# jatinchowdhury18/differentiable-wdfs

Hardware: AMD Instinct MI355X
Metric: samples/sec fwd+bwd, 1N4148 diode clipper @48kHz batch=8192; 1->8 GPU scaling (higher is better)
Workload: dtype f32

## Files before the change

### differentiable-wdfs_amd/csrc/wdf_clipper.h

```cpp
#pragma once

#include <hip/hip_runtime.h>
#include <stdint.h>
#include <type_traits>

#include "wdf_omega.h"
#include "wdf_optim.h"

namespace wdf {

#ifdef WDF_DBG_TIMES
__device__ unsigned long long* g_dbg_times = nullptr;
#define WDF_DBG_STAMP(i)                                                                                     \
    do { if (threadIdx.x == 0 && g_dbg_times)                                                                \
             g_dbg_times[8 * ((size_t)gridDim.x * gridDim.y) + 8 * (size_t)blockIdx.x + (i)] = wall_clock64(); } while (0)
#else
#define WDF_DBG_STAMP(i) do {} while (0)
#endif

constexpr int kBlk = 8;

struct ClipConsts {
    float Is, V;
    float G2;
// ... 78 lines not shown
}

template <int NSTEP, bool VEC4>
__device__ __forceinline__ void load_row(const float* __restrict__ x, int64_t b, int64_t T, int64_t t0,
                                         float (&v)[NSTEP])
{
    if constexpr (VEC4) {
        const float4* p = reinterpret_cast<const float4*>(x + b * T + t0);
#pragma unroll
        for (int i = 0; i < NSTEP / 4; ++i) {
            const float4 f = p[i];
            v[4 * i] = f.x; v[4 * i + 1] = f.y; v[4 * i + 2] = f.z; v[4 * i + 3] = f.w;
        }
    } else {
#pragma unroll
        for (int k = 0; k < NSTEP; ++k) v[k] = x[b * T + t0 + k];
    }
}

template <bool TIME_MAJOR>
__device__ __forceinline__ float load_one(const float* __restrict__ x, int64_t b, int64_t B, int64_t T, int64_t t)
{
    return TIME_MAJOR ? x[t * B + b] : x[b * T + t];
}

__device__ __forceinline__ bool series_only_omega1(const ClipConsts& c)
{
    return c.L - fminf(c.d.l_up, c.d.l_dn) <= kSeriesOnlyBelow;
}

template <int DYN_R>
__device__ __forceinline__ bool fast_root_ok(const ClipConsts& c, int general)
{
    if (general) return false;
    if constexpr (DYN_R) return (c.lIV - logf(c.G2)) - fminf(c.d.l_up, c.d.l_dn) <= kSeriesOnlyBelow;
    else return series_only_omega1(c);
}

template <int DYN_R, bool SYM>
__device__ __forceinline__ int root_tier(const ClipConsts& c, int general)
{
    if (!fast_root_ok<DYN_R>(c, general)) return kRootGeneral;
    if constexpr (SYM && !DYN_R) {
        const float l0 = c.L - c.d.l_dn;
        if (l0 <= -7.5f && l0 >= -80.0f) return kRootLean;
    }
    if constexpr (SYM && DYN_R == 2) {
        const float lmax = (c.lIV - logf(c.G2)) - c.d.l_dn;
        if (lmax <= -7.5f && c.lIV >= -50.0f) return kRootLean;
    }
    return kRootFast;
}

template <int DYN_R, bool SYM, typename V, int FAST = 0>
__device__ __forceinline__ V fwd_step(const ClipConsts& c, V xin, V rin, V& z)
{
    V p, Rp, L;
    step_coeffs<DYN_R, V>(c, rin, p, Rp, L);
    const V b_diff = z - xin;
    const V b_temp = -p * b_diff;
    const V a = z + b_temp;
    const DiodeOutT<V> o = diode_pair<SYM, V, FAST>(a, L, c.d);
    const V zn = o.b + b_temp;
    const V y = 0.5f * (zn + z);
    z = zn;
    return y;
}

template <int DYN_R, bool SYM, bool TIME_MAJOR, bool VEC4, bool STASH, int FAST>
__device__ __forceinline__ void clipper_fwd_body(const ClipConsts& c, const float* __restrict__ x,
                                                 const float* __restrict__ r, float* __restrict__ y,
                                                 float* __restrict__ zstash, const float* __restrict__ z0,
                                                 float* __restrict__ zT, int64_t B, int64_t T)
{
    const int64_t b_raw = (int64_t)blockIdx.x * 64 + threadIdx.x;
    const int64_t b = b_raw < B ? b_raw : B - 1;
    float z = z0 ? z0[b] : 0.0f;
    float* __restrict__ yp = y + b;
    float* __restrict__ zp = STASH ? zstash + b : nullptr;

    const int64_t nfull = T / kBlk;
    float xc[kBlk], xn[kBlk], rc[kBlk], rn[kBlk];
#pragma unroll
    for (int k = 0; k < kBlk; ++k) { xc[k] = xn[k] = 0.0f; rc[k] = rn[k] = 1.0f; }
    if (nfull > 0) {
        load_block<TIME_MAJOR, VEC4>(x, b, B, T, 0, xn);
        if constexpr (DYN_R) load_block<TIME_MAJOR, VEC4>(r, b, B, T, 0, rn);
    }
    for (int64_t blk = 0; blk < nfull; ++blk) {
        const int64_t t0 = blk * kBlk;
#pragma unroll
        for (int k = 0; k < kBlk; ++k) { xc[k] = xn[k]; if constexpr (DYN_R) rc[k] = rn[k]; }
        if (blk + 1 < nfull) {
            load_block<TIME_MAJOR, VEC4>(x, b, B, T, t0 + kBlk, xn);
            if constexpr (DYN_R) load_block<TIME_MAJOR, VEC4>(r, b, B, T, t0 + kBlk, rn);
        }
#pragma unroll
        for (int k = 0; k < kBlk; ++k) {
            if constexpr (STASH) { *zp = z; zp += B; }
            *yp = fwd_step<DYN_R, SYM, float, FAST>(c, xc[k], rc[k], z);
            yp += B;
        }
    }
    for (int64_t t = nfull * kBlk; t < T; ++t) {
        const float xin = load_one<TIME_MAJOR>(x, b, B, T, t);
        const float rin = DYN_R ? load_one<TIME_MAJOR>(r, b, B, T, t) : 1.0f;
        if constexpr (STASH) { *zp = z; zp += B; }
        *yp = fwd_step<DYN_R, SYM, float, FAST>(c, xin, rin, z);
        yp += B;
    }
    if (zT) zT[b] = z;
}

template <int DYN_R, bool SYM, bool TIME_MAJOR, bool VEC4, bool STASH>
__global__ __launch_bounds__(64) void clipper_fwd_kernel(
// ... 1051 lines not shown
```

### differentiable-wdfs_amd/csrc/wdf_clipper_fused.h

```cpp
#pragma once

#include "wdf_clipper.h"
#include "wdf_esr.h"

namespace wdf {

constexpr int kFsOut = 5;
constexpr int kFsOutEsr = 6;
constexpr int kFsPart = 4;
constexpr int kFsPartEsr = 8;
template <int LOSS> struct FusedRec {
    static constexpr int N = LOSS == 2 ? kFsOutEsr : kFsOut;
    static constexpr int NP = LOSS == 2 ? kFsPartEsr : kFsPart;
};
constexpr int kFsQuads = 3;
template <int NSEQ, int LOSS> struct FusedQuads { static constexpr int NQ = (NSEQ * FusedRec<LOSS>::N + 3) / 4; };
__device__ __forceinline__ float* rec_chunk(float* rec, int64_t k) { return rec + (size_t)k * kFsQuads * ((size_t)gridDim.x * 64) * 4; }
constexpr int kFusedSchedGroup = 1;
#ifndef WDF_FUSED_ROWS
#define WDF_FUSED_ROWS 16
#endif
#ifndef WDF_FUSED_PREFETCH_AT
#define WDF_FUSED_PREFETCH_AT 0
#endif
// ... 238 lines not shown
        const int g = threadIdx.x & 3, lr = threadIdx.x >> 2;
        commit(a);
#pragma unroll
        for (int m = 0; m < N * 2; ++m)
            *reinterpret_cast<v4u*>(lds + (o * HR + m * 16 + lr) * kWinPitch + kWinPhase + g * 4) = tail[m];
        read(tw, v);
        if (N == 1 && tw + NR < t_end) issue(o, tw + NR);
    }
    __device__ __forceinline__ void next(int64_t tn, int64_t t_end, V (&v)[NR])
    {
        const int sel = (int)(tn / kWinPhase) & 1, u = (int)(tn / NR) % N;
        if (u == 0) commit(sel);
        read(tn, v);
        if (u == N - 1 && tn + NR < t_end) issue(sel ^ 1, tn + NR);
    }
};

template <typename V>
__device__ __forceinline__ V load_own(const float* row, const LaneOwn<V>& q)
{
    V r = vsplat<V>(0.0f);
#pragma unroll
    for (int j = 0; j < VT<V>::N; ++j) vset(r, j, row[q.b + j]);
    return r;
}
template <typename V>
__device__ __forceinline__ void store_own(float* row, const LaneOwn<V>& q, V v)
{
#pragma unroll
    for (int j = 0; j < VT<V>::N; ++j) row[q.b + j] = vget(v, j);
}
template <typename V>
__device__ __forceinline__ void publish_own(float* row, const LaneOwn<V>& q, V v)
{
#pragma unroll
    for (int j = 0; j < VT<V>::N; ++j) __hip_atomic_store(row + q.b + j, vget(v, j), __ATOMIC_RELAXED, __HIP_MEMORY_SCOPE_AGENT);
}
template <typename V, bool TM>
__device__ __forceinline__ V load_step(const float* __restrict__ x, const LaneOwn<V>& q, int64_t B, int64_t T, int64_t t)
{
    V r = vsplat<V>(0.0f);
#pragma unroll
    for (int j = 0; j < VT<V>::N; ++j) vset(r, j, load_one<TM>(x, q.b + j, B, T, t));
    return r;
}

template <typename V>
struct FusedTan {
    V A, cL, cV, cP;
    V GA, GL, GV, GP;
    V hg_prev;
    V sse;
    V HA, HL, HV, HP, hy_prev, syy;
    __device__ __forceinline__ void init()
    {
        A = vsplat<V>(1.0f);
        cL = cV = cP = GA = GL = GV = GP = hg_prev = sse = vsplat<V>(0.0f);
        HA = HL = HV = HP = hy_prev = syy = vsplat<V>(0.0f);
    }
    template <int LOSS>
    __device__ __forceinline__ void pin()
    {
        vpin(A); vpin(cL); vpin(cV); vpin(cP); vpin(GA); vpin(GL); vpin(GV); vpin(GP); vpin(sse);
        if constexpr (LOSS == 2) { vpin(HA); vpin(HL); vpin(HV); vpin(HP); vpin(syy); }
    }
};

template <int DYN_R, bool SYM, int FAST, typename V, int LOSS = 1>
__device__ __forceinline__ V fused_step(const ClipConsts& c, V xin, V rin, V tgt, float hgs, V& z, FusedTan<V>& s)
{
    V p, Rp, L;
    step_coeffs<DYN_R, V>(c, rin, p, Rp, L);
    const V b_diff = z - xin;
    const V b_temp = -p * b_diff;
    const V a = z + b_temp;
    const DiodeOutT<V> o = diode_pair<SYM, V, FAST>(a, L, c.d);
    const V zn = o.b + b_temp;
    const V y = 0.5f * (zn + z);
    const V w0p = o.w0 * vrcp(o.w0 + 1.0f);
    V Da, DL, DV;
    if constexpr (SYM && FAST == kRootLean && !DYN_R) {
        const V w1p = vfma(-o.w1, o.w1, o.w1);
        const V sp = w0p + w1p;
        const V tl = vsel_nonzero(a, -2.0f, 0.0f);
        const float tvm = c.d.two_v * c.d.m_dn;
        Da = vfma(tl, sp, 1.0f);
        DL = vcopysign(w0p - w1p, a);
        DV = vfma(tl * a, sp, tvm * vcopysign(o.dw, a));
        const V cPl = vfma(-Da, b_diff, -b_diff);
        const V kappa_l = vfma(Da, 1.0f - c.p, -c.p);
        const V d = y - tgt;
        const V hg = hgs * d;
        s.sse = vfma(hg, d, s.sse);
        const V hh = hg + s.hg_prev;
        s.hg_prev = hg;
        s.GA = vfma(hh, s.A, s.GA);
        s.GL = vfma(hh, s.cL, s.GL);
        s.GV = vfma(hh, s.cV, s.GV);
        s.GP = vfma(hh, s.cP, s.GP);
        if constexpr (LOSS == 2) {
            const V hy = hgs * y;
            s.syy = vfma(hy, y, s.syy);
            const V h2 = hy + s.hy_prev;
            s.hy_prev = hy;
            s.HA = vfma(h2, s.A, s.HA);
            s.HL = vfma(h2, s.cL, s.HL);
            s.HV = vfma(h2, s.cV, s.HV);
            s.HP = vfma(h2, s.cP, s.HP);
        }
        s.A = s.A * kappa_l;
        s.cL = vfma(kappa_l, s.cL, DL);
        s.cV = vfma(kappa_l, s.cV, DV);
        s.cP = vfma(kappa_l, s.cP, cPl);
        z = zn;
        return y;
    } else
    if constexpr (SYM && FAST) {
        V w1p;
        if constexpr (FAST == kRootLean) w1p = vfma(-o.w1, o.w1, o.w1);
        else w1p = o.w1 * vfma(-o.w1, vfma(-o.w1, 1.0f - o.w1, 1.0f), 1.0f);
        const V sp = w0p + w1p;
        const V tl = vsel_nonzero(a, -2.0f, 0.0f);
        const float tvm = c.d.two_v * c.d.m_dn;
        Da = vfma(tl, sp, 1.0f);
        DL = (-tvm) * vcopysign(w0p - w1p, a);
        DV = vfma(tl * a, sp * (-1.0f / c.V), (-2.0f * c.d.m_dn) * vcopysign(o.dw, a));
    } else {
        const V w1p = o.w1 * vrcp(o.w1 + 1.0f);
        const V l2 = o.lam * o.lam;
        const V sp = w0p + w1p;
        const V tl = -2.0f * l2;
        Da = vfma(tl, sp, 1.0f);
        if constexpr (SYM) {
            const float tvm = c.d.two_v * c.d.m_dn;
            DL = (-tvm) * (o.lam * (w0p - w1p));
            DV = vfma(tl * a, sp * (-1.0f / c.V), (-2.0f * c.d.m_dn) * (o.lam * (o.w0 - o.w1)));
        } else {
            DL = (-c.d.two_v) * (o.lam * (o.m0 * w0p - o.m1 * w1p));
            DV = vfma(tl * a, sp * (-1.0f / c.V), -2.0f * (o.lam * (o.m0 * o.w0 - o.m1 * o.w1)));
        }
    }
    const V opd = Da + 1.0f;
    V cP = -opd * b_diff;
    if constexpr (DYN_R) cP = Rp * vfma(cP, p, DL);
    const V kappa = vfma(-p, opd, Da);
    const V d = y - tgt;
    const V hg = hgs * d;
    s.sse = vfma(hg, d, s.sse);
    const V hh = hg + s.hg_prev;
    s.hg_prev = hg;
    s.GA = vfma(hh, s.A, s.GA);
    s.GL = vfma(hh, s.cL, s.GL);
    s.GV = vfma(hh, s.cV, s.GV);
    s.GP = vfma(hh, s.cP, s.GP);
    if constexpr (LOSS == 2) {
        const V hy = hgs * y;
        s.syy = vfma(hy, y, s.syy);
        const V h2 = hy + s.hy_prev;
        s.hy_prev = hy;
        s.HA = vfma(h2, s.A, s.HA);
        s.HL = vfma(h2, s.cL, s.HL);
        s.HV = vfma(h2, s.cV, s.HV);
        s.HP = vfma(h2, s.cP, s.HP);
    }
    s.A = s.A * kappa;
    s.cL = vfma(kappa, s.cL, DL);
// ... 109 lines not shown
    int64_t t0, t1;
    chunk_span(k, K, L, skew, T, t0, t1);
    int64_t tw = 0;
    V z = vsplat<V>(0.0f);
    TpCtl c0 = {};
    if (ctl != nullptr) c0 = *ctl;
    __builtin_amdgcn_sched_barrier(0);
    const bool stateful = ctl != nullptr && c0.geom == tp_geom_tag(K, J, tp_span_scheme(skew));
    const int valid = stateful ? c0.valid : 0;
    const int head = stateful ? c0.head : 0;
    const bool warm_start = k > 0 && valid > 0 && !(stateful && c0.cold_hold > 0);
    const int jw = warm_start ? c0.j_next : 0;
    if (warm_start) tw = t0 - (int64_t)kWarmStep * jw;
    else tw = (t0 > W) ? t0 - W : 0;
    float* __restrict__ snapw = (snap != nullptr && k + 1 < K) ? snap + ((int64_t)((head + 1) % kTpRing) * J * K + k) * B : nullptr;

    const uint32_t rowb = (uint32_t)B * 4u;
    const uint32_t boff = q.boff;
    V xc[NR], xn[NR], rc[NR], rn[NR], gc[NR], gn[NR];
#pragma unroll
    for (int i = 0; i < NR; ++i) { xc[i] = xn[i] = gc[i] = gn[i] = vsplat<V>(0.0f); rc[i] = rn[i] = vsplat<V>(1.0f); }
    const int64_t nfull_end = t1 - (t1 - tw) % NR;
    constexpr bool WIN = fused_x_window<DYN_R, TM, VEC4>();
    XWindow<V, WIN> xw(x, q, B, T);
    if constexpr (WIN) static_assert(NR == XWindow<V, true>::NR, "a window is N tiles");
    if (tw < nfull_end) {
        if constexpr (WIN) xw.first_issue(tw);
        else load_x_tile<V, TM, VEC4, NR>(x, q, B, T, tw, rowb, xn);
        if constexpr (DYN_R == 1) load_x_tile<V, TM, VEC4, NR>(r, q, B, T, tw, rowb, rn);
        if constexpr (LOSS != 0) { if (tw >= t0) load_rows<V, NR>(target + tw * B, boff, rowb, gn); }
    }
    if (warm_start) {
        const int h2 = valid > 1 ? (head + kTpRing - 1) % kTpRing : head;
        const int h3 = valid > 2 ? (head + kTpRing - 2) % kTpRing : h2;
        z = load_own<V>(snap + (((int64_t)head * J + jw) * K + (k - 1)) * B, q);
        const V z2 = load_own<V>(snap + (((int64_t)h2 * J + jw) * K + (k - 1)) * B, q);
        const V z3 = load_own<V>(snap + (((int64_t)h3 * J + jw) * K + (k - 1)) * B, q);
        __builtin_amdgcn_sched_barrier(0);
        if (valid > 1) {
            const TpExtrap e = tp_extrapolation(theta, c0, valid);
            const V zs = vfma(vsplat<V>(e.lam), z - z2, z);
            if (e.quad) {
                const V zq = vfma(vsplat<V>(e.w3), z3 - z, vfma(vsplat<V>(e.w2), z2 - z, z));
                const V c = zq - zs;
                z = zs + vsel(vgt_c(vabs(c), 4.0e-7f), c, vsplat<V>(0.0f));
            } else {
                z = zs;
            }
        }
    } else if (tw == 0 && z0) {
        z = load_own<V>(z0, q);
    }
    int64_t t = tw;
    if constexpr (WIN) { if (tw < nfull_end) xw.first(tw, nfull_end, xn); }
#ifdef WDF_DBG_TIMES
    dbg_p[1] = __builtin_amdgcn_s_memtime();
#endif
    for (; t < t0 && t < nfull_end; t += NR) {
#pragma unroll
        for (int i = 0; i < NR; ++i) { xc[i] = xn[i]; if constexpr (DYN_R == 1) rc[i] = rn[i]; }
        if (t + NR < nfull_end) {
            if constexpr (WIN) xw.next(t + NR, nfull_end, xn);
            else load_x_tile<V, TM, VEC4, NR>(x, q, B, T, t + NR, rowb, xn);
            if constexpr (DYN_R == 1) load_x_tile<V, TM, VEC4, NR>(r, q, B, T, t + NR, rowb, rn);
            if constexpr (LOSS != 0) { if (t + NR >= t0) load_rows<V, NR>(target + (t + NR) * B, boff, rowb, gn); }
        }
#pragma unroll
        for (int i = 0; i < NR; ++i) (void)fwd_step<DYN_R, SYM, V, FAST>(c, xc[i], rc[i], z);
    }
#ifdef WDF_DBG_TIMES
    dbg_p[2] = __builtin_amdgcn_s_memtime();
#endif
    publish_own<V>(zwarm + k * B, q, z);
    if (gs != nullptr) {
#pragma unroll
        for (int j = 0; j < VT<V>::N; ++j) gs->zin[j][threadIdx.x & 63u] = vget(z, j);
    }
    wait_vmcnt<0>();
#ifdef WDF_DBG_TIMES
    dbg_p[3] = __builtin_amdgcn_s_memtime();
#endif
    FusedTan<V> s;
    s.init();
    FusedSums<V> d;
    d.init();
#ifdef WDF_DBG_TIMES
    unsigned long long dbg_wait = 0;
#endif
    for (; t < nfull_end; t += NR) {
#pragma unroll
        for (int i = 0; i < NR; ++i) { xc[i] = xn[i]; gc[i] = gn[i]; if constexpr (DYN_R == 1) rc[i] = rn[i]; }
        const bool more = t + NR < nfull_end;
        if (snapw != nullptr && t1 - t <= (int64_t)kWarmStep * (J - 1) && (t1 - t) % kWarmStep == 0)
            store_own<V>(snapw + ((t1 - t) / kWarmStep) * K * B, q, z);
        [[maybe_unused]] const __amdgpu_buffer_rsrc_t ry = row_rsrc(STORE_Y ? y + t * B : nullptr);
        [[maybe_unused]] const __amdgpu_buffer_rsrc_t rz = row_rsrc(STASH ? zstash + t * B : (STORE_Y ? y + t * B : nullptr));
        const int64_t below = skip - t;
        const int n_masked = __builtin_amdgcn_readfirstlane((int)(below < 0 ? 0 : (below > NR ? NR : below)));
#pragma unroll
        for (int i = 0; i < NR; ++i) {
            if (i == kFusedPrefetchAt * NR / 2) {
                __builtin_amdgcn_sched_barrier(0);
                if (more) {
                    if constexpr (WIN) xw.next(t + NR, nfull_end, xn);
                    else load_x_tile<V, TM, VEC4, NR>(x, q, B, T, t + NR, rowb, xn);
                    if constexpr (DYN_R == 1) load_x_tile<V, TM, VEC4, NR>(r, q, B, T, t + NR, rowb, rn);
                    if constexpr (LOSS != 0) load_rows<V, NR>(target + (t + NR) * B, boff, rowb, gn);
                }
                __builtin_amdgcn_sched_barrier(0);
            }
            if constexpr (LOSS == 0) {
                if constexpr (STASH) buf_store_nt(z, rz, boff, i * rowb);
                buf_store_nt(fwd_step<DYN_R, SYM, V, FAST>(c, xc[i], rc[i], z), ry, boff, i * rowb);
                continue;
            }
            if constexpr (STORE_Y)
                buf_store_nt(fused_step<DYN_R, SYM, FAST, V, LOSS>(c, xc[i], rc[i], gc[i], step_loss_scale(i, n_masked, hgs), z, s), ry, boff,
                             i * rowb);
            else
                (void)fused_step<DYN_R, SYM, FAST, V, LOSS>(c, xc[i], rc[i], gc[i], step_loss_scale(i, n_masked, hgs), z, s);
            if (i % kFusedSchedGroup == kFusedSchedGroup - 1) {
                s.template pin<LOSS>();
                __builtin_amdgcn_sched_barrier(0);
            }
        }
#ifdef WDF_DBG_TIMES
        { const unsigned long long w0 = __builtin_amdgcn_s_memtime(); wait_vmcnt<NR>(); dbg_wait += __builtin_amdgcn_s_memtime() - w0; }
#else
        wait_vmcnt<STORE_Y ? NR * (STASH ? 2 : 1) : 0>();
#endif
        if constexpr (LOSS != 0) { if ((t + NR - t0) % kFlushSteps == 0) d.template flush<LOSS>(s); }
    }
    for (int64_t tt = nfull_end; tt < t1; ++tt) {
        const V xin = load_step<V, TM>(x, q, B, T, tt);
        const V rin = DYN_R == 1 ? load_step<V, TM>(r, q, B, T, tt) : vsplat<V>(1.0f);
        if constexpr (LOSS == 0) {
            if constexpr (STASH) store_own<V>(zstash + tt * B, q, z);
            store_own<V>(y + tt * B, q, fwd_step<DYN_R, SYM, V, FAST>(c, xin, rin, z));
            continue;
        }
        const V tg = load_own<V>(target + tt * B, q);
        if constexpr (STORE_Y) store_own<V>(y + tt * B, q, fused_step<DYN_R, SYM, FAST, V, LOSS>(c, xin, rin, tg, tt >= skip ? hgs : 0.0f, z, s));
        else (void)fused_step<DYN_R, SYM, FAST, V, LOSS>(c, xin, rin, tg, tt >= skip ? hgs : 0.0f, z, s);
    }
    d.template flush<LOSS>(s);
    publish_own<V>(zend + k * B, q, z);
    if (gs != nullptr) {
#pragma unroll
        for (int j = 0; j < VT<V>::N; ++j) gs->zend[j][threadIdx.x & 63u] = vget(z, j);
    }
    if (snapw != nullptr) store_own<V>(snapw, q, z);
    if (zT && t1 == T) store_own<V>(zT, q, z);
    if constexpr (LOSS != 0) {
        FusedScale fsc{1.0f, 1.0f};
        if constexpr (SYM && FAST == kRootLean && !DYN_R) fsc = FusedScale{-(c.d.two_v * c.d.m_dn), -1.0f / c.V};
        fused_publish_record<V, LOSS, VT<V>::N>(rec, wpart, k, K, q.live, 0, s, d, hgs, fsc, gs != nullptr ? &gs->rec[0][0] : nullptr,
                                                gs != nullptr ? gs->part : nullptr);
    }
#ifdef WDF_DBG_TIMES
    dbg_p[4] = __builtin_amdgcn_s_memtime();
    if ((threadIdx.x & 63u) == 0 && g_dbg_times) {
        unsigned long long* o = g_dbg_times + 8 * ((size_t)k * gridDim.x + blockIdx.x);
        o[2] = dbg_wait;
        o[4] = dbg_p[1] - dbg_p[0]; o[5] = dbg_p[2] - dbg_p[1]; o[6] = dbg_p[3] - dbg_p[2]; o[7] = dbg_p[4] - dbg_p[3];
    }
#endif
}

struct FusedOut {
    float* gtheta; int accumulate; float* sse_out; AdamTail adam;
    double n_global, eps; float* sums10; float* loss3;
    TpFinishCtx fc;
};

template <bool REDUCED = false>
__device__ __forceinline__ void esr_tile_partial_and_finish(const double (&v)[8], double* ws, unsigned* gticket, const float* theta,
                                                            float fs, int dyn_r, const FusedOut& out)
{
    const unsigned ntiles = gridDim.x;
    double w[8];
#pragma unroll
    for (int i = 0; i < 8; ++i) w[i] = REDUCED ? v[i] : wave_sum_dpp(v[i]);
    unsigned done = 0;
    if (threadIdx.x == 0) {
        double* o = ws + (int64_t)blockIdx.x * 8;
#pragma unroll
        for (int i = 0; i < 8; ++i) __hip_atomic_store(o + i, w[i], __ATOMIC_RELAXED, __HIP_MEMORY_SCOPE_AGENT);
        asm volatile("s_waitcnt vmcnt(0)" ::: "memory");
        done = atomicAdd(&gticket[0], 1u);
    }
    done = __builtin_amdgcn_readfirstlane(done);
    if (done != ntiles - 1) return;
    if (threadIdx.x == 0) gticket[0] = 0u;
    double t[8] = {0.0, 0.0, 0.0, 0.0, 0.0, 0.0, 0.0, 0.0};
    for (unsigned i = threadIdx.x; i < ntiles; i += 64)
#pragma unroll
// ... 283 lines not shown
    TpStatus* __restrict__ status, TpCtl* ctl, float* snap, int J, unsigned* tickets, float tol, int64_t B,
    int64_t Bh, int64_t T, int64_t L, int64_t W, int general, int verify_later)
{
    static_assert(VT<V>::N == 1, "one sequence per lane (the repair kernel and tp_finish index tiles of 64)");
#ifdef WDF_DBG_TIMES
    const unsigned long long dbg_t0 = wall_clock64();
    const unsigned long long dbg_m0 = __builtin_amdgcn_s_memtime();
#endif
    if (verify_later && blockIdx.x == 0 && blockIdx.y == 0 && threadIdx.x == 0) *status = TpStatus{0, 0.0f, 0, 0u};
    const ClipConsts c = load_consts(theta, fs, n_up, n_down);
    const int tier = root_tier<DYN_R, SYM>(c, general);
    bool ran = false;
    if constexpr (SYM && DYN_R != 1) {
        if (tier == kRootLean) {
            clipper_fused_body<DYN_R, SYM, TM, VEC4, kRootLean, V, 0, STASH>(c, x, r, nullptr, y, zstash, z0, zT, zwarm, zend, nullptr, theta,
                                                                             ctl, snap, J, B, T, L, W, 0.0f, 0, blockIdx.y, gridDim.y);
            ran = true;
        }
    }
    if (!ran) {
        if (tier != kRootGeneral)
            clipper_fused_body<DYN_R, SYM, TM, VEC4, kRootFast, V, 0, STASH>(c, x, r, nullptr, y, zstash, z0, zT, zwarm, zend, nullptr, theta,
                                                                             ctl, snap, J, B, T, L, W, 0.0f, 0, blockIdx.y, gridDim.y);
        else
            clipper_fused_body<DYN_R, SYM, TM, VEC4, kRootGeneral, V, 0, STASH>(c, x, r, nullptr, y, zstash, z0, zT, zwarm, zend, nullptr, theta,
                                                                                ctl, snap, J, B, T, L, W, 0.0f, 0, blockIdx.y, gridDim.y);
    }
#ifdef WDF_DBG_TIMES
    if (threadIdx.x == 0 && g_dbg_times) {
        unsigned long long* dbg_o = g_dbg_times + 8 * ((size_t)blockIdx.y * gridDim.x + blockIdx.x);
        dbg_o[0] = dbg_t0; dbg_o[1] = wall_clock64(); dbg_o[3] = __builtin_amdgcn_s_memtime() - dbg_m0;
        dbg_o[2] = (unsigned long long)__builtin_amdgcn_s_getreg((4 << 0) | (0 << 6) | (31 << 11)) |
                   ((unsigned long long)__builtin_amdgcn_s_getreg((20 << 0) | (0 << 6) | (31 << 11)) << 32);
    }
#endif
    if (!verify_later) tp_finish<DYN_R>(theta, zwarm, zend, status, ctl, J, tickets, tol, B, L, W);
#ifdef WDF_DBG_TIMES
    if (threadIdx.x == 0 && g_dbg_times) g_dbg_times[8 * ((size_t)blockIdx.y * gridDim.x + blockIdx.x) + 4] = wall_clock64();
#endif
}

template <int DYN_R, bool SYM, bool TM, int FAST, int LOSS, int NSEQ, bool STORE_Y = true>
__device__ __forceinline__ void fused_rerun_chunk(const ClipConsts& c_in, const float* __restrict__ x, const float* __restrict__ r,
                                                  const float* __restrict__ target, float* __restrict__ y, float* rec, double* wpart,
                                                  float* __restrict__ snapw, int J, int64_t K, int64_t k, int64_t b, int64_t B,
                                                  bool live, int slot, int64_t T, int64_t t0, int64_t t1, float hgs, int64_t skip,
                                                  float& z)
{
    const ClipConstsSeq<float> c = make_seq_consts<DYN_R, float>(c_in, DYN_R == 2 ? load_one<TM>(r, b, B, T, 0) : 1.0f);
    FusedTan<float> s;
    s.init();
    FusedSums<float> d;
    d.init();
    for (int64_t t = t0; t < t1; t += kBlk) {
        if ((t - t0) % kWarmStep == 0) {
            d.template flush<LOSS>(s);
            if (snapw != nullptr && t1 - t <= (int64_t)kWarmStep * (J - 1) && (t1 - t) % kWarmStep == 0)
                snapw[((t1 - t) / kWarmStep) * K * B + b] = z;
        }
        float xv[kBlk], rv[kBlk], gv[kBlk];
#pragma unroll
        for (int i = 0; i < kBlk; ++i) {
            const int64_t tt = (t + i < t1) ? t + i : t1 - 1;
            xv[i] = load_one<TM>(x, b, B, T, tt);
            rv[i] = DYN_R == 1 ? load_one<TM>(r, b, B, T, tt) : 1.0f;
            gv[i] = target[tt * B + b];
        }
#pragma unroll
        for (int i = 0; i < kBlk; ++i) {
            if (t + i < t1) {
                if constexpr (STORE_Y)
                    y[(t + i) * B + b] = fused_step<DYN_R, SYM, FAST, float, LOSS>(c, xv[i], rv[i], gv[i], (t + i >= skip) ? hgs : 0.0f, z, s);
                else
                    (void)fused_step<DYN_R, SYM, FAST, float, LOSS>(c, xv[i], rv[i], gv[i], (t + i >= skip) ? hgs : 0.0f, z, s);
            }
        }
    }
    d.template flush<LOSS>(s);
    if (snapw != nullptr) snapw[b] = z;
    FusedScale fsc{1.0f, 1.0f};
    if constexpr (SYM && FAST == kRootLean && !DYN_R) fsc = FusedScale{-(c.d.two_v * c.d.m_dn), -1.0f / c.V};
    fused_publish_record<float, LOSS, NSEQ>(rec, wpart, k, K, live, slot, s, d, hgs, fsc);
}

template <int DYN_R, bool SYM, bool TM, int NSEQ, int LOSS>
__global__ __launch_bounds__(64) void clipper_fused_repair_kernel(
    const float* __restrict__ x, const float* __restrict__ r, const float* theta, float fs, int n_up, int n_down,
    const float* __restrict__ target, float hgs, int64_t skip, float* __restrict__ y, float* __restrict__ zT,
    const float* zwarm, float* zend, float* rec, int64_t B, int64_t T, int64_t K, int64_t L, float tol,
    TpStatus* __restrict__ status, TpCtl* ctl, float* __restrict__ snap, int J, unsigned* tickets,
    unsigned* gticket, int general, double* ws, FusedOut out, int64_t skew, double* wpart, int64_t W)
{
    __shared__ double sh[64][4];
    unsigned* tile_bad = tickets + 4 + gridDim.x;
    if (tile_bad[blockIdx.x] == 0u) return;
    const int64_t raw = ((int64_t)blockIdx.x * 64 + threadIdx.x) * NSEQ;
    const bool live = raw < B;
    const int64_t b0 = live ? raw : B - NSEQ;
    const ClipConsts c = load_consts(theta, fs, n_up, n_down);
    const int tier = root_tier<DYN_R, SYM>(c, general);
    int slot = 0;
    if (ctl != nullptr && snap != nullptr) slot = ((ctl->geom == tp_geom_tag(K, J, tp_span_scheme(skew)) ? ctl->head : 0) + 1) % kTpRing;
    int nrep = 0;
#pragma unroll 1
    for (int h = 0; h < NSEQ; ++h) {
        const int64_t b = b0 + h;
        bool fixed_prev = false;
        float ze_fix = 0.0f;
        for (int64_t k = 1; k < K; ++k) {
            const float e = fixed_prev ? ze_fix : load_published(zend + (k - 1) * B + b);
            const float m = fabsf(load_published(zwarm + k * B + b) - e);
            fixed_prev = false;
            if (__builtin_amdgcn_ballot_w64(!(m <= tol)) == 0) continue;
            int64_t t0, t1;
            chunk_span(k, K, L, skew, T, t0, t1);
            float* __restrict__ snapw = (snap != nullptr && k + 1 < K) ? snap + ((int64_t)slot * J * K + k) * B : nullptr;
            float z = e;
            bool ran = false;
            if constexpr (SYM && DYN_R != 1) {
                if (tier == kRootLean) {
                    fused_rerun_chunk<DYN_R, SYM, TM, kRootLean, LOSS, NSEQ>(c, x, r, target, y, rec, wpart, snapw, J, K, k, b, B, live, h, T, t0, t1, hgs, skip, z);
                    ran = true;
                }
            }
            if (!ran) {
                if (tier != kRootGeneral) fused_rerun_chunk<DYN_R, SYM, TM, kRootFast, LOSS, NSEQ>(c, x, r, target, y, rec, wpart, snapw, J, K, k, b, B, live, h, T, t0, t1, hgs, skip, z);
                else fused_rerun_chunk<DYN_R, SYM, TM, kRootGeneral, LOSS, NSEQ>(c, x, r, target, y, rec, wpart, snapw, J, K, k, b, B, live, h, T, t0, t1, hgs, skip, z);
// ... 434 lines not shown
```

### differentiable-wdfs_amd/csrc/wdf_omega.h

```cpp
#pragma once

#include <hip/hip_runtime.h>

#include "wdf_vec.h"

namespace wdf {

constexpr float kLog2e = 1.4426950408889634f;
constexpr float kLn2 = 0.6931471805599453f;
constexpr float kRegion4Hi = 4.141592653589793f;

__device__ __forceinline__ float fast_exp(float x) { return __builtin_amdgcn_exp2f(x * kLog2e); }
__device__ __forceinline__ float fast_log(float x) { return __builtin_amdgcn_logf(x) * kLn2; }
__device__ __forceinline__ float fast_rcp(float x) { return __builtin_amdgcn_rcpf(x); }

template <typename V>
__device__ __forceinline__ V fsc_step(V x, V w, V& r)
{
    r = vfma(vlog2(w), -kLn2, x - w);
    const V wp1 = w + 1.0f;
    const V tmr = vfma(wp1 + wp1, vfma(r, 2.0f / 3.0f, wp1), -r);
    const V e = (r * tmr) * vrcp(wp1 * (tmr - r));
    return vfma(w, e, w);
}

constexpr float kSeriesOnlyBelow = -4.0f;

constexpr float kSecondIterResidual = 0.05f;

template <typename V>
__device__ __forceinline__ V omega_series_of_exp(V p)
{
    return p * vfma(p, vfma(p, vfma(p, vfma(p, 125.0f / 24.0f, -8.0f / 3.0f), 1.5f), -1.0f), 1.0f);
}

template <typename V>
__device__ __forceinline__ V omega_series(V x)
{
    return omega_series_of_exp(vexp2(vmin_c(x, -2.0f) * kLog2e));
}

template <typename V>
__device__ __forceinline__ V omega_series_unclamped(V x)
{
    return omega_series_of_exp(vexp2(x * kLog2e));
}

template <typename V>
__device__ __forceinline__ V omega_start(V x)
{
    V wA = omega_series_unclamped(x);
    const V q = x - 1.0f;
    const V sB = vfma(q, vfma(q, vfma(q, 13.0f / 61440.0f, -1.0f / 3072.0f), -1.0f / 192.0f), 1.0f / 16.0f);
    V wB = vfma(sB, q * q, vfma(x, 0.5f, 0.5f));
    const V lg = vlog2(x);
    const V l = lg * kLn2;
    V wC = vfma(l, vrcp(x), vfma(lg, -kLn2, x));
    vpin(wA); vpin(wB); vpin(wC);
    return vsel(vle_c(x, -2.0f), wA, vsel(vle_c(x, kRegion4Hi), wB, wC));
}

template <typename V>
__device__ __forceinline__ V omega_one_step(V x, typename VT<V>::mask& again)
{
    const V w0 = omega_start(x);
    V r;
    V w1 = fsc_step(x, w0, r);
    vpin(w1);
    const auto refine = vgt_c(x, kSeriesOnlyBelow);
    again = mand(refine, vge_c(vabs(r), kSecondIterResidual));
    return vsel(refine, w1, w0);
}

template <typename V>
__device__ __forceinline__ V omega_second_step(V x, V w, typename VT<V>::mask again)
{
    V r2;
    const V w2 = fsc_step(x, vsel(again, w, vsplat<V>(1.0f)), r2);
    return vsel(again, w2, w);
}

template <bool COUNT_ITERS = false>
__device__ __forceinline__ float wright_omega(float x, int* iters = nullptr)
{
    bool again;
    float w = omega_one_step<float>(x, again);
    if (__builtin_amdgcn_ballot_w64(again)) w = omega_second_step<float>(x, w, again);
    if constexpr (COUNT_ITERS) { if (iters) *iters = (x > kSeriesOnlyBelow ? 1 : 0) + (again ? 1 : 0); }
    return w;
}

template <typename V>
__device__ __forceinline__ V omega_lean(V x)
{
    const V p = vexp2(x * kLog2e);
    V wA = vfma(-p, p, p);
    const V q = x - 1.0f;
    const V sB = vfma(q, vfma(q, vfma(q, 13.0f / 61440.0f, -1.0f / 3072.0f), -1.0f / 192.0f), 1.0f / 16.0f);
    V wB = vfma(sB, q * q, vfma(x, 0.5f, 0.5f));
    const V lg = vlog2(x);
    const V l = lg * kLn2;
    V wC = vfma(l, vrcp(x), vfma(lg, -kLn2, x));
    vpin(wA); vpin(wB); vpin(wC);
    const V w0 = vsel(vle_c(x, -2.0f), wA, vsel(vle_c(x, kRegion4Hi), wB, wC));
    V r;
    return fsc_step(x, w0, r);
}

constexpr int kRootGeneral = 0, kRootFast = 1, kRootLean = 2;

struct DiodeStatic {
    float i_up, i_dn;
    float l_up, l_dn;
    float m_up, m_dn;
    float two_v;
};

__device__ __forceinline__ DiodeStatic make_diode_static(float nVt, int n_up, int n_down)
{
    DiodeStatic c;
    c.m_up = (float)n_up;
    c.m_dn = (float)n_down;
    c.i_up = 1.0f / (c.m_up * nVt);
    c.i_dn = 1.0f / (c.m_dn * nVt);
    c.l_up = logf(c.m_up);
    c.l_dn = logf(c.m_dn);
    c.two_v = 2.0f * nVt;
    return c;
}

template <typename V>
struct DiodeOutT {
    V b;
    V w0, w1;
    V lam;
    V m0, m1;
    V dw;
};
using DiodeOut = DiodeOutT<float>;

template <bool SYM, typename V, int TIER = 0>
__device__ __forceinline__ DiodeOutT<V> diode_pair(V a, V L, const DiodeStatic& c)
{
    constexpr bool FAST = TIER >= kRootFast;
    constexpr bool LEAN = TIER == kRootLean && SYM;
    DiodeOutT<V> o;
    o.lam = vsign(a);
    const V aa = vabs(a);
    V u0, u1, e1 = vsplat<V>(0.0f);
    if constexpr (SYM) {
        o.m0 = o.m1 = vsplat<V>(c.m_dn);
        const V l0 = L - c.l_dn;
        u0 = vfma(aa, c.i_dn, l0);
        u1 = vfma(aa, -c.i_dn, l0);
        e1 = vfma(aa, -c.i_dn * kLog2e, l0 * kLog2e);
    } else {
        const auto pos = vge_c(a, 0.0f);
        o.m0 = vsel(pos, c.m_dn, c.m_up);
        o.m1 = vsel(pos, c.m_up, c.m_dn);
        const V i0 = vsel(pos, c.i_dn, c.i_up), i1 = vsel(pos, c.i_up, c.i_dn);
        const V l0 = L - vsel(pos, c.l_dn, c.l_up), l1 = L - vsel(pos, c.l_up, c.l_dn);
        u0 = vfma(aa, i0, l0);
        u1 = l1 - aa * i1;
    }
    typename VT<V>::mask again0{};
    if constexpr (LEAN) o.w0 = omega_lean<V>(u0);
    else o.w0 = omega_one_step<V>(u0, again0);
    if constexpr (LEAN) {
        const V p1 = vexp2(e1);
        o.w1 = vfma(-p1, p1, p1);
        vpin(o.w1);
    } else if constexpr (FAST && SYM) {
        o.w1 = omega_series_of_exp<V>(vexp2(e1));
        vpin(o.w1);
    } else {
        o.w1 = omega_series<V>(u1);
    }
    if constexpr (!FAST) {
        const auto general1 = vgt_c(u1, kSeriesOnlyBelow);
        if (__builtin_amdgcn_ballot_w64(many(mor(again0, general1)))) {
            o.w0 = omega_second_step<V>(u0, o.w0, again0);
            typename VT<V>::mask again1;
            V w1g = omega_one_step<V>(u1, again1);
            w1g = omega_second_step<V>(u1, w1g, again1);
            o.w1 = vsel(general1, w1g, o.w1);
        }
    }
    o.dw = o.w0 - o.w1;
    if constexpr (LEAN) o.dw = vsel_nz(a, o.dw);
    if constexpr (SYM && FAST) o.b = a - (c.two_v * c.m_dn) * vcopysign(o.dw, a);
    else if constexpr (SYM) o.b = a - (c.two_v * c.m_dn) * (o.lam * (o.w0 - o.w1));
    else o.b = a - c.two_v * (o.lam * (o.m0 * o.w0 - o.m1 * o.w1));
    return o;
}

}
```

Baseline: 366.6 billion.

## Use lane-table ds_bpermute initial guess for omega and defer tangent updates

Replaces the three-branch polynomial/log initial guess in the lean Wright-omega path with a 64-entry piecewise-linear table held one entry per lane and read with ds_bpermute, indexed by the float exponent/mantissa bits of the shifted input. A slow fallback covers large inputs. It also defers the tangent/gradient accumulation of each step so it runs in the latency shadow of the next step's cross-lane gathers, which overlaps LDS-permute latency with arithmetic. The costs are extra registers for pending state, table setup per thread, and dependence on the table being accurate enough for the single refinement step.

```diff
diff --git a/differentiable-wdfs_amd/csrc/wdf_clipper.h b/differentiable-wdfs_amd/csrc/wdf_clipper.h
--- a/differentiable-wdfs_amd/csrc/wdf_clipper.h
+++ b/differentiable-wdfs_amd/csrc/wdf_clipper.h
@@ -154,15 +154,15 @@
     return kRootFast;
 }
 
-template <int DYN_R, bool SYM, typename V, int FAST = 0>
-__device__ __forceinline__ V fwd_step(const ClipConsts& c, V xin, V rin, V& z)
+template <int DYN_R, bool SYM, typename V, int FAST = 0, typename TAB = OmegaNoTab>
+__device__ __forceinline__ V fwd_step(const ClipConsts& c, V xin, V rin, V& z, const TAB& tab = TAB{})
 {
     V p, Rp, L;
     step_coeffs<DYN_R, V>(c, rin, p, Rp, L);
     const V b_diff = z - xin;
     const V b_temp = -p * b_diff;
     const V a = z + b_temp;
-    const DiodeOutT<V> o = diode_pair<SYM, V, FAST>(a, L, c.d);
+    const DiodeOutT<V> o = diode_pair<SYM, V, FAST, TAB>(a, L, c.d, tab);
     const V zn = o.b + b_temp;
     const V y = 0.5f * (zn + z);
     z = zn;
diff --git a/differentiable-wdfs_amd/csrc/wdf_clipper_fused.h b/differentiable-wdfs_amd/csrc/wdf_clipper_fused.h
--- a/differentiable-wdfs_amd/csrc/wdf_clipper_fused.h
+++ b/differentiable-wdfs_amd/csrc/wdf_clipper_fused.h
@@ -314,11 +314,37 @@
     V hg_prev;
     V sse;
     V HA, HL, HV, HP, hy_prev, syy;
+    V p_hh, p_h2, p_k, p_L, p_V, p_P;
     __device__ __forceinline__ void init()
     {
         A = vsplat<V>(1.0f);
         cL = cV = cP = GA = GL = GV = GP = hg_prev = sse = vsplat<V>(0.0f);
         HA = HL = HV = HP = hy_prev = syy = vsplat<V>(0.0f);
+        p_hh = p_h2 = p_k = p_L = p_V = p_P = vsplat<V>(0.0f);
+    }
+    template <int LOSS>
+    __device__ __forceinline__ void apply_pending()
+    {
+        GA = vfma(p_hh, A, GA);
+        GL = vfma(p_hh, cL, GL);
+        GV = vfma(p_hh, cV, GV);
+        GP = vfma(p_hh, cP, GP);
+        if constexpr (LOSS == 2) {
+            HA = vfma(p_h2, A, HA);
+            HL = vfma(p_h2, cL, HL);
+            HV = vfma(p_h2, cV, HV);
+            HP = vfma(p_h2, cP, HP);
+        }
+        A = A * p_k;
+        cL = vfma(p_k, cL, p_L);
+        cV = vfma(p_k, cV, p_V);
+        cP = vfma(p_k, cP, p_P);
+    }
+    template <int LOSS>
+    __device__ __forceinline__ void pin_pending()
+    {
+        vpin(p_hh); vpin(p_k); vpin(p_L); vpin(p_V); vpin(p_P);
+        if constexpr (LOSS == 2) vpin(p_h2);
     }
     template <int LOSS>
     __device__ __forceinline__ void pin()
@@ -328,15 +354,20 @@
     }
 };
 
-template <int DYN_R, bool SYM, int FAST, typename V, int LOSS = 1>
-__device__ __forceinline__ V fused_step(const ClipConsts& c, V xin, V rin, V tgt, float hgs, V& z, FusedTan<V>& s)
+constexpr int kTanNow = 0, kTanDeferFirst = 1, kTanDefer = 2;
+
+template <int DYN_R, bool SYM, int FAST, typename V, int LOSS = 1, typename TAB = OmegaNoTab>
+__device__ __forceinline__ V fused_step(const ClipConsts& c, V xin, V rin, V tgt, float hgs, V& z, FusedTan<V>& s, const TAB& tab = TAB{},
+                                        int defer = kTanNow)
 {
     V p, Rp, L;
     step_coeffs<DYN_R, V>(c, rin, p, Rp, L);
     const V b_diff = z - xin;
     const V b_temp = -p * b_diff;
     const V a = z + b_temp;
-    const DiodeOutT<V> o = diode_pair<SYM, V, FAST>(a, L, c.d);
+    const DiodeOutT<V> o = diode_pair<SYM, V, FAST, TAB>(a, L, c.d, tab, [&]() {
+        if (defer == kTanDefer) { s.template pin_pending<LOSS>(); s.template apply_pending<LOSS>(); s.template pin<LOSS>(); }
+    });
     const V zn = o.b + b_temp;
     const V y = 0.5f * (zn + z);
     const V w0p = o.w0 * vrcp(o.w0 + 1.0f);
@@ -354,26 +385,19 @@
         const V d = y - tgt;
         const V hg = hgs * d;
         s.sse = vfma(hg, d, s.sse);
-        const V hh = hg + s.hg_prev;
+        s.p_hh = hg + s.hg_prev;
         s.hg_prev = hg;
-        s.GA = vfma(hh, s.A, s.GA);
-        s.GL = vfma(hh, s.cL, s.GL);
-        s.GV = vfma(hh, s.cV, s.GV);
-        s.GP = vfma(hh, s.cP, s.GP);
         if constexpr (LOSS == 2) {
             const V hy = hgs * y;
             s.syy = vfma(hy, y, s.syy);
-            const V h2 = hy + s.hy_prev;
+            s.p_h2 = hy + s.hy_prev;
             s.hy_prev = hy;
-            s.HA = vfma(h2, s.A, s.HA);
-            s.HL = vfma(h2, s.cL, s.HL);
-            s.HV = vfma(h2, s.cV, s.HV);
-            s.HP = vfma(h2, s.cP, s.HP);
-        }
-        s.A = s.A * kappa_l;
-        s.cL = vfma(kappa_l, s.cL, DL);
-        s.cV = vfma(kappa_l, s.cV, DV);
-        s.cP = vfma(kappa_l, s.cP, cPl);
+        }
+        s.p_k = kappa_l;
+        s.p_L = DL;
+        s.p_V = DV;
+        s.p_P = cPl;
+        if (defer == kTanNow) s.template apply_pending<LOSS>();
         z = zn;
         return y;
     } else
@@ -589,6 +613,9 @@
         z = load_own<V>(z0, q);
     }
     int64_t t = tw;
+    constexpr bool TABLE = kOmegaTable && LOSS != 0 && SYM && FAST == kRootLean;
+    typename std::conditional<TABLE, OmegaTab, OmegaNoTab>::type tab{};
+    if constexpr (TABLE) tab = omega_tab_fill();
     if constexpr (WIN) { if (tw < nfull_end) xw.first(tw, nfull_end, xn); }
 #ifdef WDF_DBG_TIMES
     dbg_p[1] = __builtin_amdgcn_s_memtime();
@@ -603,7 +630,7 @@
             if constexpr (LOSS != 0) { if (t + NR >= t0) load_rows<V, NR>(target + (t + NR) * B, boff, rowb, gn); }
         }
 #pragma unroll
-        for (int i = 0; i < NR; ++i) (void)fwd_step<DYN_R, SYM, V, FAST>(c, xc[i], rc[i], z);
+        for (int i = 0; i < NR; ++i) (void)fwd_step<DYN_R, SYM, V, FAST>(c, xc[i], rc[i], z, tab);
     }
 #ifdef WDF_DBG_TIMES
     dbg_p[2] = __builtin_amdgcn_s_memtime();
@@ -651,16 +678,20 @@
                 buf_store_nt(fwd_step<DYN_R, SYM, V, FAST>(c, xc[i], rc[i], z), ry, boff, i * rowb);
                 continue;
             }
+            constexpr bool DEFER = TABLE && !DYN_R;
+            const int defer = !DEFER ? kTanNow : (i == 0 ? kTanDeferFirst : kTanDefer);
             if constexpr (STORE_Y)
-                buf_store_nt(fused_step<DYN_R, SYM, FAST, V, LOSS>(c, xc[i], rc[i], gc[i], step_loss_scale(i, n_masked, hgs), z, s), ry, boff,
-                             i * rowb);
+                buf_store_nt(fused_step<DYN_R, SYM, FAST, V, LOSS>(c, xc[i], rc[i], gc[i], step_loss_scale(i, n_masked, hgs), z, s, tab, defer), ry,
+                             boff, i * rowb);
             else
-                (void)fused_step<DYN_R, SYM, FAST, V, LOSS>(c, xc[i], rc[i], gc[i], step_loss_scale(i, n_masked, hgs), z, s);
+                (void)fused_step<DYN_R, SYM, FAST, V, LOSS>(c, xc[i], rc[i], gc[i], step_loss_scale(i, n_masked, hgs), z, s, tab, defer);
             if (i % kFusedSchedGroup == kFusedSchedGroup - 1) {
                 s.template pin<LOSS>();
+                if constexpr (DEFER) s.template pin_pending<LOSS>();
                 __builtin_amdgcn_sched_barrier(0);
             }
         }
+        if constexpr (LOSS != 0 && TABLE && !DYN_R) s.template apply_pending<LOSS>();
 #ifdef WDF_DBG_TIMES
         { const unsigned long long w0 = __builtin_amdgcn_s_memtime(); wait_vmcnt<NR>(); dbg_wait += __builtin_amdgcn_s_memtime() - w0; }
 #else
@@ -677,8 +708,8 @@
             continue;
         }
         const V tg = load_own<V>(target + tt * B, q);
-        if constexpr (STORE_Y) store_own<V>(y + tt * B, q, fused_step<DYN_R, SYM, FAST, V, LOSS>(c, xin, rin, tg, tt >= skip ? hgs : 0.0f, z, s));
-        else (void)fused_step<DYN_R, SYM, FAST, V, LOSS>(c, xin, rin, tg, tt >= skip ? hgs : 0.0f, z, s);
+        if constexpr (STORE_Y) store_own<V>(y + tt * B, q, fused_step<DYN_R, SYM, FAST, V, LOSS>(c, xin, rin, tg, tt >= skip ? hgs : 0.0f, z, s, tab));
+        else (void)fused_step<DYN_R, SYM, FAST, V, LOSS>(c, xin, rin, tg, tt >= skip ? hgs : 0.0f, z, s, tab);
     }
     d.template flush<LOSS>(s);
     publish_own<V>(zend + k * B, q, z);
@@ -1068,6 +1099,9 @@
     s.init();
     FusedSums<float> d;
     d.init();
+    constexpr bool TABLE = kOmegaTable && SYM && FAST == kRootLean;
+    typename std::conditional<TABLE, OmegaTab, OmegaNoTab>::type tab{};
+    if constexpr (TABLE) tab = omega_tab_fill();
     for (int64_t t = t0; t < t1; t += kBlk) {
         if ((t - t0) % kWarmStep == 0) {
             d.template flush<LOSS>(s);
@@ -1086,9 +1120,9 @@
         for (int i = 0; i < kBlk; ++i) {
             if (t + i < t1) {
                 if constexpr (STORE_Y)
-                    y[(t + i) * B + b] = fused_step<DYN_R, SYM, FAST, float, LOSS>(c, xv[i], rv[i], gv[i], (t + i >= skip) ? hgs : 0.0f, z, s);
+                    y[(t + i) * B + b] = fused_step<DYN_R, SYM, FAST, float, LOSS>(c, xv[i], rv[i], gv[i], (t + i >= skip) ? hgs : 0.0f, z, s, tab);
                 else
-                    (void)fused_step<DYN_R, SYM, FAST, float, LOSS>(c, xv[i], rv[i], gv[i], (t + i >= skip) ? hgs : 0.0f, z, s);
+                    (void)fused_step<DYN_R, SYM, FAST, float, LOSS>(c, xv[i], rv[i], gv[i], (t + i >= skip) ? hgs : 0.0f, z, s, tab);
             }
         }
     }
diff --git a/differentiable-wdfs_amd/csrc/wdf_omega.h b/differentiable-wdfs_amd/csrc/wdf_omega.h
--- a/differentiable-wdfs_amd/csrc/wdf_omega.h
+++ b/differentiable-wdfs_amd/csrc/wdf_omega.h
@@ -1,6 +1,8 @@
 #pragma once
 
 #include <hip/hip_runtime.h>
+
+#include <type_traits>
 
 #include "wdf_vec.h"
 
@@ -91,7 +93,7 @@
 }
 
 template <typename V>
-__device__ __forceinline__ V omega_lean(V x)
+__device__ __forceinline__ V omega_lean_start(V x)
 {
     const V p = vexp2(x * kLog2e);
     V wA = vfma(-p, p, p);
@@ -102,7 +104,64 @@
     const V l = lg * kLn2;
     V wC = vfma(l, vrcp(x), vfma(lg, -kLn2, x));
     vpin(wA); vpin(wB); vpin(wC);
-    const V w0 = vsel(vle_c(x, -2.0f), wA, vsel(vle_c(x, kRegion4Hi), wB, wC));
+    return vsel(vle_c(x, -2.0f), wA, vsel(vle_c(x, kRegion4Hi), wB, wC));
+}
+
+template <typename V>
+__device__ __forceinline__ V omega_lean(V x)
+{
+    const V w0 = omega_lean_start(x);
+    V r;
+    return fsc_step(x, w0, r);
+}
+
+#ifndef WDF_OMEGA_TABLE
+#define WDF_OMEGA_TABLE 1
+#endif
+constexpr bool kOmegaTable = WDF_OMEGA_TABLE != 0;
+constexpr float kOmegaTabShift = 3.0f;
+constexpr float kOmegaTabEnd = 253.0f;
+struct OmegaNoTab {};
+struct OmegaNoFill { __device__ __forceinline__ void operator()() const {} };
+struct OmegaTab { float c0, c1; };
+
+__device__ __forceinline__ OmegaTab omega_tab_fill()
+{
+    const unsigned j = ((threadIdx.x & 63u) + 8u) & 63u;
+    const float t_lo = __uint_as_float(0x3F800000u + (j << 20)), t_hi = __uint_as_float(0x3F800000u + ((j + 1u) << 20));
+    const float w_lo = wright_omega(t_lo - kOmegaTabShift), w_hi = wright_omega(t_hi - kOmegaTabShift);
+    const float w_mid = wright_omega(0.5f * (t_lo + t_hi) - kOmegaTabShift);
+    OmegaTab tab;
+    tab.c1 = (w_hi - w_lo) / (t_hi - t_lo);
+    tab.c0 = (w_lo - tab.c1 * t_lo) + 0.5f * (w_mid - 0.5f * (w_lo + w_hi));
+    return tab;
+}
+
+template <typename V> struct OmegaGather { V t, c0, c1; };
+
+__device__ __forceinline__ float omega_tab_gather(float t, float v)
+{
+    return __int_as_float(__builtin_amdgcn_ds_bpermute((int)(__float_as_uint(t) >> 18), __float_as_int(v)));
+}
+__device__ __forceinline__ OmegaGather<float> omega_tab_issue(float x, const OmegaTab& tab)
+{
+    const float t = x + kOmegaTabShift;
+    return OmegaGather<float>{t, omega_tab_gather(t, tab.c0), omega_tab_gather(t, tab.c1)};
+}
+__device__ __forceinline__ OmegaGather<v2f> omega_tab_issue(v2f x, const OmegaTab& tab)
+{
+    const v2f t = x + kOmegaTabShift;
+    return OmegaGather<v2f>{t, v2f{omega_tab_gather(t.x, tab.c0), omega_tab_gather(t.y, tab.c0)},
+                            v2f{omega_tab_gather(t.x, tab.c1), omega_tab_gather(t.y, tab.c1)}};
+}
+
+template <typename V>
+__device__ __forceinline__ V omega_tab_finish(V x, const OmegaGather<V>& g, V wA)
+{
+    V ws = vfma(g.c1, g.t, g.c0);
+    vpin(wA); vpin(ws);
+    V w0 = vsel(vle_c(x, -2.0f), wA, ws);
+    if (__builtin_amdgcn_ballot_w64(many(vge_c(x, kOmegaTabEnd)))) w0 = omega_lean_start(x);
     V r;
     return fsc_step(x, w0, r);
 }
@@ -139,8 +198,8 @@
 };
 using DiodeOut = DiodeOutT<float>;
 
-template <bool SYM, typename V, int TIER = 0>
-__device__ __forceinline__ DiodeOutT<V> diode_pair(V a, V L, const DiodeStatic& c)
+template <bool SYM, typename V, int TIER = 0, typename TAB = OmegaNoTab, typename FILL = OmegaNoFill>
+__device__ __forceinline__ DiodeOutT<V> diode_pair(V a, V L, const DiodeStatic& c, const TAB& tab = TAB{}, FILL fill = FILL{})
 {
     constexpr bool FAST = TIER >= kRootFast;
     constexpr bool LEAN = TIER == kRootLean && SYM;
@@ -164,9 +223,22 @@
         u1 = l1 - aa * i1;
     }
     typename VT<V>::mask again0{};
-    if constexpr (LEAN) o.w0 = omega_lean<V>(u0);
+    constexpr bool TABLE = LEAN && std::is_same<TAB, OmegaTab>::value;
+    if constexpr (TABLE) {
+        const OmegaGather<V> g = omega_tab_issue(u0, tab);
+        __builtin_amdgcn_sched_barrier(0);
+        fill();
+        const V p0 = vexp2(u0 * kLog2e);
+        const V wA = vfma(-p0, p0, p0);
+        const V p1 = vexp2(e1);
+        o.w1 = vfma(-p1, p1, p1);
+        vpin(o.w1);
+        __builtin_amdgcn_sched_barrier(0);
+        o.w0 = omega_tab_finish(u0, g, wA);
+    } else if constexpr (LEAN) o.w0 = omega_lean<V>(u0);
     else o.w0 = omega_one_step<V>(u0, again0);
-    if constexpr (LEAN) {
+    if constexpr (TABLE) {
+    } else if constexpr (LEAN) {
         const V p1 = vexp2(e1);
         o.w1 = vfma(-p1, p1, p1);
         vpin(o.w1);
```

Result: no change. 365.5 billion (-0.3%).
